# Photoroom/datago

Measured on AMD Instinct MI355X. Metric: Mpixel/s device-resident JPEG decode+bucket-resize at 1/2/4/8 MI355X, higher is better.
Workload: dtype u8

## Files before the change

datago_amd/csrc/dg_entropy.h:

```cpp
#pragma once
#include "dg_pixel.h"
#include "dg_plane.h"
#include "dg_types.h"

namespace dg {

DG_HD int32_t huff_extend(int32_t v, int32_t s) { return v < (1 << (s - 1)) ? v - (1 << s) + 1 : v; }

DG_HD uint32_t bswap32(uint32_t x) {
  return (x >> 24) | ((x >> 8) & 0xFF00u) | ((x << 8) & 0xFF0000u) | (x << 24);
}

DG_HD uint32_t ds_word_index(uint32_t w, uint32_t lsw) {
  const uint32_t s = w >> lsw, j = w & ((1u << lsw) - 1u);
  return ((((s >> 6) << lsw) + j) << 6) + (s & 63u);
}
DG_HD uint64_t ds_words_alloc(uint32_t nsub, uint32_t lsw) {
  const uint32_t margin = ((1024u >> 5) >> lsw) + 2u;
  return ((uint64_t)((nsub + margin + 63u) / 64u) << lsw) * 64;
}

constexpr uint32_t kBwBuf = 6;

struct BitWin {
// ... 369 lines not shown
}
DG_HD DG_GLOBAL uint32_t *stage_range(uint64_t stage, uint32_t cap, uint32_t s) {
  return (DG_GLOBAL uint32_t *)(uintptr_t)stage + ((((size_t)(s >> 6) * cap) << 6) + (s & 63u)) * 4;
}
DG_HD void stage_push(StageCtx &c, uint32_t e) {
  const uint32_t k = c.n & 3u;
  c.g0 = k == 0 ? e : c.g0;
  c.g1 = k == 1 ? e : c.g1;
  c.g2 = k == 2 ? e : c.g2;
  c.g3 = k == 3 ? e : c.g3;
  c.n++;
  if (k == 3) {
    DG_GLOBAL uint32_t *p = c.base + (size_t)((c.n >> 2) - 1) * 256;
#if defined(DG_DEVICE)
    *(DG_GLOBAL u32x4 *)p = u32x4{c.g0, c.g1, c.g2, c.g3};
#else
    p[0] = c.g0, p[1] = c.g1, p[2] = c.g2, p[3] = c.g3;
#endif
  }
}
DG_HD void stage_finish(StageCtx &c) {
  if (c.n & 3u) {
    DG_GLOBAL uint32_t *p = c.base + (size_t)(c.n >> 2) * 256;
#if defined(DG_DEVICE)
    *(DG_GLOBAL u32x4 *)p = u32x4{c.g0, c.g1, c.g2, c.g3};
#else
    p[0] = c.g0, p[1] = c.g1, p[2] = c.g2, p[3] = c.g3;
#endif
  }
}

constexpr uint32_t kCkptBits = 256;
constexpr uint32_t kMaxCkpt = 16;
template <int NC>
struct CkptN {
  uint32_t st;
  uint32_t m, n;
  int32_t dc[NC];
};
using Ckpt = CkptN<3>;

DG_HD uint32_t num_ckpt(uint32_t sub_bits) {
  uint32_t k = (sub_bits - 1) / kCkptBits;
  return k > kMaxCkpt ? kMaxCkpt : k;
}

DG_HD uint32_t first_marker(const DG_GLOBAL uint32_t *mk, uint32_t nmk, uint32_t pos, uint32_t &idx) {
  uint32_t lo = 0, hi = nmk;
  while (lo < hi) {
    uint32_t mid = (lo + hi) >> 1;
    if (mk[mid] < pos) lo = mid + 1;
    else hi = mid;
  }
  idx = lo;
  return lo < nmk ? mk[lo] : kInf;
}

template <class TAB>
DG_HD uint32_t lead_in(const ImageDesc &im, const TAB *tabs, const DG_GLOBAL uint8_t *stream,
                       const DG_GLOBAL uint32_t *mk, uint32_t s, uint32_t lead,
                       const uint16_t *mt = nullptr, uint32_t acm = 0xFFu, bool pair = false, uint32_t chain = 0) {
  const uint32_t a0 = s * im.sub_bits;
  if (s == 0 || lead == 0 || a0 >= im.ds_bits) return pack_state(0, 0, 0);
  uint32_t pos = a0 > lead ? a0 - lead : 0u;
  uint32_t r = 0, z = 0, midx;
  uint32_t mpos = im.nmk ? first_marker(mk, im.nmk, pos, midx) : kInf;
  const uint32_t bpm = im.bpm, slotmap = im.slotmap, cbits = im.comp_bits;
  uint32_t comp = cbits & 3u;
  const TAB *tdc = &tabs[(slotmap >> ((comp << 1) << 2)) & 15u];
  const TAB *tac = &tabs[(slotmap >> (((comp << 1) | 1u) << 2)) & 15u];
  uint32_t mi = mt ? (acm >> (2u * comp)) & 3u : 3u;
  BitWin b;
  bw_init(b, stream, im.ds_lsw, pos);
  for (;;) {
    if (pos >= mpos) {
      pos = mpos;
      r = 0;
// ... 127 lines not shown
          setn(acc.dc, 0);
          if (WRITE) {
            w->seg++;
            w->nin = 0;
            setn(w->pred, 0);
          }
        }
        midx++;
        mpos = midx < im.nmk ? mk[midx] : kInf;
        bw_seek(b, pos);
      }
      if (k < nck && cpos < a1 && pos >= cpos) {
        uint32_t rel = pos - cpos;
        uint32_t st = pack_state(rel > 255 ? 255 : rel, r, z);
        DG_GLOBAL CkptN<NC> &c = ck[k];
        if (merge && c.st == st) {
          if (c.m) {
            acc.m += c.m;
            acc.n = c.n;
            cpyn<NC>(acc.dc, c.dc);
          } else {
            acc.n += c.n;
            accn<NC>(acc.dc, c.dc);
          }
          acc.out = old_out;
          merged = true;
          break;
        }
        c.st = st;
        c.m = acc.m;
        c.n = acc.n;
        cpyn<NC>(c.dc, acc.dc);
        k++;
        cpos += kCkptBits;
      }
      if (pos >= a1) break;
      ev = next_event();
    }
    bw_refill(b);
    const uint32_t bits = bw_peek(b, pos);
    const bool isdc = (z == 0);
    const uint32_t e = huff_decode(*(isdc ? tdc : tac), bits);
    const uint32_t len = e >> 8, sym = e & 0xFFu;
    const uint32_t size = sym & 15u;
    const uint32_t run = isdc ? 0u : (sym >> 4);
    const int32_t v = huff_value(bits, len, size);
    uint32_t zm = 0xFFFFFFFFu, mc = 0;
    if (!WRITE) {
      const uint32_t m = (mi != 3u && !isdc) ? (uint32_t)mt[(mi << kMultiBits) | (bits >> (32u - kMultiBits))] : 0u;
      mc = m & 15u;
      zm = pos + mc <= ev ? multi_next_z(m, z) : 0xFFFFFFFFu;
    }
    const bool take_m = zm != 0xFFFFFFFFu;
    const uint32_t p0 = pos;
    pos += take_m ? mc : len + size;
    const int32_t vdc = isdc ? v : 0;
    acc.n += isdc ? 1u : 0u;
    addn(acc.dc, comp, vdc);
    if (stage) {
      if (isdc) {
        stg->started++;
        if (v) stage_push(*stg, stage_coef(0, stg->started, v));
      } else if (size && z + run < 64) {
        stage_push(*stg, stage_coef(z + run, stg->started, v));
      }
    }
    if (WRITE) {
// ... 309 lines not shown
```

datago_amd/csrc/dg_types.h:

```cpp
#pragma once
#include <stdint.h>

#if defined(__HIP__)
#define DG_HD __host__ __device__ __forceinline__
#define DG_DEVICE 1
#define DG_GLOBAL __attribute__((address_space(1)))
typedef unsigned int u32x4 __attribute__((ext_vector_type(4)));
typedef unsigned int u32x2 __attribute__((ext_vector_type(2)));
#else
#define DG_HD static inline
#define DG_GLOBAL
#endif

namespace dg {

template <class T>
DG_HD DG_GLOBAL T *gp(uint64_t a) {
  return (DG_GLOBAL T *)(uintptr_t)a;
}

DG_HD int32_t sel3(const int32_t v[3], uint32_t c) { return c == 0 ? v[0] : (c == 1 ? v[1] : v[2]); }
DG_HD void add3(int32_t v[3], uint32_t c, int32_t d) {
  v[0] += c == 0 ? d : 0;
  v[1] += c == 1 ? d : 0;
// ... 448 lines not shown
  uint32_t first;
  uint32_t next;
  uint64_t deps;
};
constexpr uint32_t kProgDone = 0xFFFFFFFFu;
constexpr uint32_t kProgNoScan = 0xFFFFFFFFu;
constexpr uint16_t kProgChained = 1;
constexpr uint32_t kProgMaxScans = 256;
constexpr uint32_t kProgMaxDepScans = 64;
constexpr uint32_t kProgZeroBytes = 65536;

struct WgItem {
  uint32_t image;
  uint32_t item0;
};

struct BatchFlags {
  uint32_t chain_changed;
  uint32_t fix_count;
  uint32_t write_mismatch;
  uint32_t sync_iters_max;
  uint32_t idct_late;
  uint32_t png_next;
  uint64_t wgtime;
  uint32_t wgtime_write;
  uint32_t debug;
  uint64_t idct_list;
  uint32_t idct_cap;
  uint32_t prio;
};
constexpr size_t kFlagCounters = 24;
constexpr uint32_t kDbgForceWriteMismatch = 1u;
constexpr uint32_t kDbgForceChainChange = 2u;

}
```

datago_amd/csrc/host/options.cpp:

```cpp
#include "options.h"

#include <string.h>

namespace dg {

static_assert(sizeof(size_t) == sizeof(uint64_t), "size_t fields are kOptU64");
static_assert(kMaxInflight == 6, "the texts of \"slots\" and \"coalesce_inflight\" spell it out");

namespace {

template <class T> constexpr OptType opt_type();
template <> constexpr OptType opt_type<bool>() { return kOptBool; }
template <> constexpr OptType opt_type<int>() { return kOptInt; }
template <> constexpr OptType opt_type<uint32_t>() { return kOptU32; }
template <> constexpr OptType opt_type<int64_t>() { return kOptI64; }
template <> constexpr OptType opt_type<uint64_t>() { return kOptU64; }
template <> constexpr OptType opt_type<double>() { return kOptDouble; }

constexpr int64_t kNoMax = INT64_MAX;

#define DG_STR2(x) #x
#define DG_STR(x) DG_STR2(x)
#define F(f) offsetof(Options, f), opt_type<decltype(Options::f)>()
#define FLAG(key, f) {key, F(f), kOptFlag, 0, 0, 0, 0, nullptr, kAfterNone}
// ... 66 lines not shown
    RANGE("decode_semantics", decode_sem, 0, 1, "valid unless v != 0 && v != 1"),
    RANGE("small_coded", small_coded, 0, kNoMax, "valid unless v < 0"),
    POW2("sub_small", sub_small, 64, 65536, "valid unless v < 64 || v > 65536 || (v & (v - 1))"),
    RANGE("lead_small", lead_small, 0, 1 << 16, "valid unless v < 0 || v > (1 << 16)"),
    POW2_OR_0("v_tile", v_tile, 2, 8, "valid: 0, 2, 4, 8"),
    RANGE("v_units", v_units, 1, 8, "valid unless v < 1 || v > 8"),
    RANGE("lead_big", lead_big, 0, 1 << 16, "valid unless v < 0 || v > (1 << 16)"),
    FLAG("write_split", write_split),
    RANGE("meta_pull", meta_pull, 0, 2, "valid unless v < 0 || v > 2"),
    RANGE("plan_threads", plan_threads, 1, 64, "valid unless v < 1 || v > 64"),
    POW2("inf_stage3", inf_stage3, 8, 64, "valid unless v != 8 && v != 16 && v != 32 && v != 64"),
    RANGE("inf_cap", inf_cap, 10, 100, "valid unless v < 10 || v > 100"),
    FLAG("png_alias", png_alias),
    RANGE("inf_pad", inf_pad, 0, 1 << 20, "valid unless v < 0 || v > 2^20"),
    POW2("inf_chunk", inf_chunk, 4096, 65536, "valid unless v < 4096 || v > 65536 || (v & (v - 1))"),
    {"png_chunked", F(chunked_off), kOptFlagInv, 0, 0, 0, 0, nullptr, kAfterNone},
    FLAG("lead_density", lead_density),
    RANGE("sub_density", sub_density, 0, 4096, "valid unless v < 0 || v > 4096"),
    RANGE("uf_per_cu", uf_per_cu, 0, 16, "valid unless v < 0 || v > 16"),
    RANGE("uf_units", uf_units, 1, 2, "valid unless v < 1 || v > 2"),
    {"inf_decode", F(inf_decode), kOptRangeBut, 0, 28, 10, 0, "valid unless v < 0 || v > 28 || v == 10", kAfterNone},
    FLAG("h_mfma", h_mfma),
    FLAG("band_dec", band_dec),
    RAW("dec_dbg", dec_dbg),
    RANGE("dec_strips", dec_strips, 1, 4096, "valid unless v < 1 || v > 4096"),
    RAW("debug_flags", debug_flags),
};
const int kNumOptions = (int)(sizeof(kOptionTable) / sizeof(kOptionTable[0]));

const OptRow kOptionTableAdded[] = {
    STRICT("webp_lossy", webp_lossy),
    STRICT("webp_alpha", webp_alpha),
    STRICT("bmp", bmp),
};
const int kNumOptionsAdded = (int)(sizeof(kOptionTableAdded) / sizeof(kOptionTableAdded[0]));

const OptRow *find_option(const char *key) {
  for (const OptRow &r : kOptionTable)
    if (!strcmp(r.name, key)) return &r;
  for (const OptRow &r : kOptionTableAdded)
    if (!strcmp(r.name, key)) return &r;
  return nullptr;
}

bool option_takes(const OptRow &r, int64_t v) {
  switch (r.kind) {
    case kOptRange: return v >= r.lo && v <= r.hi;
    case kOptRangeBut: return v >= r.lo && v <= r.hi && v != r.except;
    case kOptPow2: return v >= r.lo && v <= r.hi && !(v & (v - 1));
    case kOptPow2Or0: return v == 0 || (v >= r.lo && v <= r.hi && !(v & (v - 1)));
    default: return true;
  }
}

void store_option(const OptRow &r, Options &o, int64_t v) {
  void *p = (char *)&o + r.off;
  switch (r.type) {
    case kOptNone: break;
    case kOptBool: *(bool *)p = r.kind == kOptFlagInv ? v == 0 : v != 0; break;
    case kOptInt: *(int *)p = (int)v; break;
    case kOptU32: *(uint32_t *)p = (uint32_t)v; break;
    case kOptI64: *(int64_t *)p = v; break;
    case kOptU64: *(uint64_t *)p = (uint64_t)v << r.shift; break;
    case kOptDouble: *(double *)p = (double)v; break;
  }
}
// ... 21 lines not shown
```

datago_amd/csrc/host/options.h:

```cpp
#pragma once
#include <stddef.h>
#include <stdint.h>

#include <string>

#include "../dg_types.h"

namespace dg {

constexpr int kMaxInflight = 6;
#ifndef DG_PROG_SLOTS
#define DG_PROG_SLOTS 2
#endif
constexpr int kProgSlots = DG_PROG_SLOTS;

struct Options {
  uint32_t sub_bits = 0;
  uint32_t sub_auto = 8192;
  int64_t lead_bits = -1;
  uint32_t lead_big = 4096;
  uint64_t small_coded = 0;
  uint32_t sub_small = 512, lead_small = 1024;
  double sub_density = 0;
  bool lead_density = false;
  bool multi_lead = true;
  int write_pair = 3;
  bool sync2 = false;
  int sync_chain = 2;
  bool sync_pair = false;
  bool write_split = true;
  bool ckpt = true;
  int entropy_prio = 0;
  bool entropy_lpt = true;
  bool entropy_once = false;
  bool destuff_one = false;
  int decode_sem = 0;

  bool idct_fused = false;
  bool idct_thread = true;
  bool sparse_coef = true;
  bool chroma_rec = true;
  bool band_dec = false;
  uint32_t dec_dbg = 0;
  uint32_t dec_strips = kDecStripsDefault;
  uint32_t hb_bands = kHBandsDefault;
  bool hv_fused = false;
  bool h_prefetch = true;
  bool h_planar = true;
  bool h_mfma = false;
  uint32_t v_tile = 4;
  uint32_t v_units = 2;
  size_t ccache_cap = (size_t)256 << 20;

  bool chunked_off = false;
  uint32_t inf_chunk = kInfChunk;
  uint32_t inf_cap = 30;
  bool png_alias = true;
  uint32_t inf_pad = 65536;
  uint32_t inf_stage3 = 32;
  uint32_t inf_decode = 25;
  int uf_per_cu = 0;
  uint32_t uf_units = 1;

// ... 94 lines not shown
```

datago_amd/csrc/host/pipeline.cpp:

```cpp
#include "pipeline_util.h"

#include <string.h>

#include <algorithm>
#include <atomic>
#include <chrono>
#include <cmath>
#include <thread>

#include "../dg_entropy.h"
#include "../dg_pixel.h"
#include "../dg_vp8.h"
#include "../kernels.h"

namespace dg {

thread_local std::string g_last_error;
void set_error(const std::string &s) { g_last_error = s; }

static constexpr int kMaxResyncRounds = 64;

void parallel_copy(const std::vector<CopyJob> &jobs, int nthreads) {
  constexpr size_t kPiece = 1 << 20;
  std::vector<CopyJob> pieces;
// ... 293 lines not shown
    case kAfterResetHostUs:
      for (double &x : host_us_) x = 0;
      for (double &x : host_cpu_us_) x = 0;
      break;
    default:
      break;
  }
  return DG_OK;
}

int64_t Context::get_stat(const std::string &k) {
  if (k == "batches") return stat_batches_;
  if (k == "coalesced_batches") return stat_coalesced_batches_;
  if (k == "coalesced_images") return stat_coalesced_images_;
  if (k == "resync_rounds") return stat_resync_;
  if (k == "fix_workgroups") return stat_fix_;
  if (k == "write_mismatch") return stat_mismatch_;
  if (k == "unsettled_batches") return stat_unsettled_;
  if (k == "prog_items") return stat_prog_items_;
  if (k == "prog_aggregates") return stat_prog_aggs_;
  if (k == "prog_aggregate_images") return stat_prog_agg_images_;
  if (k == "prog_chains") return stat_prog_chains_;
  if (k == "pool_flushes") return stat_pool_flush_;
  if (k == "sync_iters_max") return stat_iters_;
  if (k == "sync_chain") return opt_.sync_chain;
  {
    static const char *kn[2] = {"sync", "write"}, *sn[4] = {"span", "mean", "p90", "max"};
    for (int a = 0; a < 2; a++)
      for (int q = 0; q < 4; q++)
        if (k == std::string("wg_") + kn[a] + "_" + sn[q]) return (int64_t)(wgstat_[a][q] * 1000.0);
  }
  if (k == "sub_bits") return last_sub_bits_;
  if (k == "sub_auto") return opt_.sub_auto;
  if (k == "coalesce_inflight") return opt_.coalesce_inflight;
  if (k == "meta_bytes") return (int64_t)last_meta_bytes_;
  if (k == "allocs") return stat_allocs_;
  if (k == "alloc_mb") return stat_alloc_mb_;
  if (k == "alloc_us") return (int64_t)stat_alloc_us_;
  if (k == "reclaims") return stat_reclaims_;
  if (k == "peak_device_mb") return stat_peak_dev_ >> 20;
  if (k == "device_mb") {
    std::lock_guard<std::mutex> lk(mu_);
    return (int64_t)(dev_footprint() >> 20);
  }
  if (k == "max_device_mb") return (int64_t)(opt_.max_dev_bytes >> 20);
  if (k == "budget_splits") return stat_budget_splits_;
  if (k == "budget_plan_mb") return (int64_t)(plan_arena_ >> 20);
  if (k == "budget_slots") return opt_.max_dev_bytes ? std::min<int64_t>(opt_.nslots, stat_budget_slots_min_) : opt_.nslots;
  if (k == "coef_cache_hits") return stat_ccache_hits_;
  if (k == "coef_cache_new") return stat_ccache_new_;
  if (k == "coef_cache_resets") return stat_ccache_resets_;
  if (k == "coef_cache_mb") return (int64_t)(ccache_off_ >> 20);
  if (k == "budget_frees") return stat_budget_frees_;
  if (k == "budget_oom") return stat_budget_oom_;
  if (k == "retire_syncs") return stat_retire_syncs_;
  if (k == "png_serial_fallbacks") return stat_png_serial_;
  if (k == "band_dec_images") return stat_band_dec_;
  if (k == "direct_d2h") return stat_direct_d2h_;
  if (k == "png_chunks") return stat_png_chunks_;
  if (k == "png_small_streams") return stat_png_small_;
  {
    static const char *pn[8] = {"plan", "pools", "layout", "lists", "upload", "h2d", "launch", "slotwait"};
    for (int q = 0; q < 8; q++) {
      if (k == std::string("host_us_") + pn[q]) return (int64_t)host_us_[q];
      if (q < 7 && k == std::string("host_cpu_us_") + pn[q]) return (int64_t)host_cpu_us_[q];
    }
// ... 922 lines not shown
  if (!from_fix && !b.pscans.empty()) {
    hipStream_t pst = pside ? sl.side : sl.st;
    launch_prog_zero(pst, dd, lst(L_PROG_ZERO), cnt(L_PROG_ZERO));
    const ProgScan *ps = (const ProgScan *)(M + b.pscan_off);
    const uint32_t prog_dbg = ((uint32_t)(opt_.debug_flags >> 19) & 1u) << 1;
    uint64_t *pt = b.ptime_off ? (uint64_t *)((char *)sl.wgt.p + b.ptime_off) : nullptr;
    if (opt_.prog_pipe) {
      uint32_t *pf = (uint32_t *)((char *)sl.scratch.p + b.pf_off);
      HIPCHK(hipMemsetAsync(pf, 0, (size_t)(b.pf_n + 2) * 4, pst));
      const uint32_t nac = cnt(L_PROG) - b.prog_dc_n, sflags = (opt_.prog_serial ? 1u : 0u) | prog_dbg;
      hipStream_t dst = pst;
      if (!pside && opt_.side_stream && b.prog_dc_n && nac) {
        HIPCHK(hipEventRecord(sl.ev_zero, pst));
        HIPCHK(hipStreamWaitEvent(sl.side, sl.ev_zero, 0));
        dst = sl.side;
        dc_side = true;
      }
      launch_prog_scan(pst, dd, ps, lst(L_PROG), nac, hp, sflags, pf, pf, pt, 1);
      launch_prog_scan(dst, dd, ps, lst(L_PROG) + nac, b.prog_dc_n, hp, sflags, pf, pf + b.pf_n + 1, pt, 4);
      if (dc_side) HIPCHK(hipEventRecord(sl.ev_prog, sl.side));
    } else {
      uint32_t at = 0;
      for (uint32_t nl : b.prog_level_n) {
        launch_prog_scan(pst, dd, ps, lst(L_PROG) + at, nl, hp, opt_.prog_serial ? 1u : 0u, nullptr, nullptr, pt, 4);
        at += nl;
      }
    }
    if (pside) HIPCHK(hipEventRecord(sl.ev_prog, sl.side));
  }
  if (next()) return DG_ERR_DEVICE;
  Ckpt *ck = (Ckpt *)((char *)sl.scratch.p + sl.ckpt_off);
  if (!from_fix)
    launch_huff_sync(sl.st, dd, lst(L_SYNC), cnt(L_SYNC), hp, subs, ck, fl, b.stage_on, b.max_slots,
                     opt_.multi_lead ? b.max_ac : 0u, opt_.sync_pair, opt_.sync2, (uint32_t)opt_.sync_chain, b.nc4);
  if (next()) return DG_ERR_DEVICE;
  launch_huff_fix(sl.st, dd, lst(L_SYNC), cnt(L_SYNC), hp, subs, ck, fl, b.stage_on, b.max_slots, b.nc4);
  if (next()) return DG_ERR_DEVICE;
  launch_huff_scan(sl.st, dm, lst(L_SCAN), cnt(L_SCAN), subs, b.nc4);
  if (next()) return DG_ERR_DEVICE;
  launch_ms_zero(sl.st, dd, lst(L_MS_ZERO), cnt(L_MS_ZERO));
  if (b.stage_on)
    launch_huff_scatter(sl.st, dd, lst(L_HUFF), cnt(L_HUFF), subs);
  else
    launch_huff_write(sl.st, dm, lst(L_HUFF), cnt(L_HUFF), hp, subs, fl, b.max_slots, qp, (uint32_t)opt_.write_pair, ck,
                      b.nc4, b.ms);
  if (next()) return DG_ERR_DEVICE;
  if (next()) return DG_ERR_DEVICE;
  if (pside || dc_side) HIPCHK(hipStreamWaitEvent(sl.st, sl.ev_prog, 0));
  if (b.any_fused) launch_idct_list(sl.st, dd, qp, fl, std::min<uint32_t>(2048u, (b.idct_cap + 31) / 32));
  if (opt_.idct_thread)
    launch_idct_t(sl.st, dd, lst(L_IDCT), cnt(L_IDCT), qp);
  else
    launch_idct(sl.st, dd, lst(L_IDCT), cnt(L_IDCT), qp);
  if (next()) return DG_ERR_DEVICE;
  launch_color(sl.st, dd, lst(L_COLOR), cnt(L_COLOR));
  launch_cmyk(sl.st, dd, lst(L_CMYK), cnt(L_CMYK));
  if (next()) return DG_ERR_DEVICE;
  HIPCHK(hipStreamWaitEvent(sl.st, sl.ev_coef, 0));
  launch_alpha(sl.st, dd, lst(L_ALPHA0), cnt(L_ALPHA0), 0 | (alpha_flags << 8));
  launch_band_dec(sl.st, dd, lst(L_DEC), b.decclass, qp, opt_.dec_strips | (opt_.dec_dbg << 16));
  launch_resize_hm(sl.st, dd, lst(L_RM0), b.hmclass[0], 0);
  launch_resize_hb(sl.st, dd, lst(L_RH0), b.hclass[0], 0, opt_.h_prefetch, opt_.h_planar, b.h_zune != 0);
  launch_resize_hv(sl.st, dd, lst(L_RHV), b.hvclass);
  launch_resize_h(sl.st, dd, lst(L_RHX0), cnt(L_RHX0), 0 | ((opt_.debug_flags & 0xFF) << 8));
  if (!from_fix) launch_r16_v(sl.st, dd, lst(L_R16V), cnt(L_R16V));
  if (next()) return DG_ERR_DEVICE;
  launch_resize_v(sl.st, dd, lst(L_RV1), cnt(L_RV1), 1, opt_.v_units);
// ... 677 lines not shown
```

datago_amd/csrc/host/pipeline.h:

```cpp
#pragma once
#include <hip/hip_runtime.h>

#include <chrono>
#include <memory>
#include <condition_variable>
#include <mutex>
#include <string>
#include <unordered_map>
#include <vector>

#include "../../../include/datago_hip.h"
#include "../dg_types.h"
#include "../dg_resize16.h"
#include "buckets.h"
#include "options.h"
#include "jpeg_header.h"
#include "gif_header.h"
#include "bmp_header.h"
#include "webp_header.h"
#include "png_header.h"
#include "jpeg_enc.h"
#include "host_pool.h"

namespace dg {
// ... 47 lines not shown
  std::vector<ImagePlan> plans;
  std::vector<ImageDesc> descs;
  std::vector<int> desc_of;
  std::vector<WgItem> lists[55];
  size_t list_off[55] = {0};
  std::vector<GatherJob> gjobs;
  size_t gjob_off = 0;
  std::vector<InfChunk> ichunks;
  size_t ichunk_off = 0;
  uint32_t uf_n = 0;
  uint32_t uf_maxbpp = 1;
  size_t uf_flags_off = 0;
  uint32_t ds_n = 0;
  size_t ds_state_off = 0;
  uint32_t pf_n = 0;
  size_t pf_off = 0;
  size_t ptime_off = 0;
  uint32_t prog_dc_n = 0;
  std::vector<uint8_t> blob;
  size_t blob_off = 0;
  bool any_png = false, any_alpha = false, any_enc = false;
  bool any_gif = false;
  bool any_webp = false;
  bool any_alph = false;
  bool any_bmp = false;
  bool any_vp8 = false;
  bool penc_dyn = false;
  bool jenc_opt = false;
  bool any_fused = false;
  uint32_t idct_cap = 0;
  uint32_t v_tile = 0;
  uint32_t h_zune = 0;
  bool stage_on = false;
  bool nc4 = false;
  bool ms = false;
  struct MsScan {
    int desc, parent;
    int image, scan;
  };
  std::vector<MsScan> ms_scans;
  struct AlphStream {
    int desc, parent;
    int image;
  };
  std::vector<AlphStream> alph_streams;
  uint32_t max_slots = 1;
  uint32_t max_ac = 0;
  size_t words_off = 0, words_bytes = 0;
  size_t enctab_off = 0;
  std::vector<ProgScan> pscans;
  size_t pscan_off = 0;
  std::vector<uint32_t> prog_level_n;
  uint32_t hclass[2][2][4] = {{{0}}};
  uint32_t hvclass[2] = {0, 0};
  uint32_t decclass[2] = {0, 0};
  uint32_t hmclass[2][2][2] = {{{0}}};
  size_t desc_off = 0, flags_off = 0;
  size_t meta_bytes = 0;
  size_t total_subs = 0;
  std::vector<uint8_t *> host_outs;
  std::vector<uint64_t> host_caps;
  std::vector<size_t> out_dev_off;
  std::vector<uint8_t> out_direct;
  std::vector<dg_payload_meta *> mptr;
  std::vector<dg_payload_meta> local_meta;
  std::vector<dg_payload_meta *> pub;
// ... 315 lines not shown
```

datago_amd/csrc/host/submit.cpp:

```cpp
#include <string.h>
#include <time.h>

#include <algorithm>
#include <chrono>
#include <cmath>

#include "../dg_alph.h"
#include "../dg_entropy.h"
#include "../dg_bmp.h"
#include "../dg_gif.h"
#include "../dg_vp8.h"
#include "../dg_vp8l.h"
#include "../dg_jenc_tree.h"
#include "../dg_pixel.h"
#include "../kernels.h"
#include "pipeline_util.h"

namespace dg {

static double thread_cpu_us() {
  timespec ts;
  clock_gettime(CLOCK_THREAD_CPUTIME_ID, &ts);
  return (double)ts.tv_sec * 1e6 + (double)ts.tv_nsec * 1e-3;
}
// ... 680 lines not shown
  }
  d.nslots = (uint8_t)nslots;
  b.max_slots = std::max<uint32_t>(b.max_slots, (uint32_t)nslots);
  if (!h.progressive && !h.multiscan) {
    uint32_t acs = 0;
    for (int c = 0; c < h.ncomp; c++) acs |= 1u << ((d.slotmap >> ((2 * c + 1) * 4)) & 15u);
    b.max_ac = std::max<uint32_t>(b.max_ac, std::min<uint32_t>((uint32_t)__builtin_popcount(acs), kMultiLuts));
  }
  if (h.progressive) {
    d.prog = (uint32_t)h.scans.size();
    if (a.host_io) bl.in_off[i] = bl.IN.take(a.lens[i] + 16, 16);
  } else if (h.multiscan) {
    d.ms.role = kMsParent;
    if (a.host_io) bl.in_off[i] = bl.IN.take(a.lens[i] + 16, 16);
  } else {
    layout_entropy(a, i, b, bl, d, o);
  }
  o.coef = bl.CO.take((size_t)d.total_blocks * 128);
  o.ccnt = (opt_.sparse_coef && opt_.idct_thread && !d.prog && !d.idct_fused && !(opt_.entropy_once && !b.nc4 && !b.ms))
               ? bl.CO.take((size_t)d.total_blocks, 64) + 1
               : 0;
  for (int c = 0; c < 4; c++) o.plane[c] = (size_t)-1;
  if (h.ncomp >= 3) d.pix_stride = (uint32_t)align_up((size_t)W * 3, 16);
}

void Context::layout_entropy(const SubmitArgs &a, int i, Batch &b, BatchLayout &bl, ImageDesc &d, Offs &o) {
  const JpegHeader &h = b.plans[i].hdr;
  layout_entropy_stream(h.scan_end - h.scan_off, b, bl, d, o);
  if (a.host_io) bl.in_off[i] = bl.IN.take(a.lens[i] + 16, 16);
}

void Context::layout_entropy_stream(size_t scan_len, Batch &b, BatchLayout &bl, ImageDesc &d, Offs &o) {
  const uint32_t sub_bits = bl.sub_bits;
  const bool once = opt_.entropy_once && !b.nc4 && !b.ms;
  d.scan_len = (uint32_t)scan_len;
  d.sub_bits = sub_bits;
  if (opt_.sub_density > 0 && opt_.sub_bits == 0) {
    const double bpb = (double)d.scan_len * 8.0 / (double)std::max<uint32_t>(1, d.total_blocks);
    if (bpb < opt_.sub_density * 0.5 && sub_bits >= 2048)
      d.sub_bits = sub_bits / 4;
    else if (bpb < opt_.sub_density && sub_bits >= 1024)
      d.sub_bits = sub_bits / 2;
  }
  d.idct_fused = (opt_.idct_fused && !once && !b.nc4 && !b.ms) ? 1u : 0u;
  if (opt_.write_split && d.ckpt && !d.idct_fused && !once && d.restart == 0 && d.sub_bits >= 1024 &&
      d.sub_bits / 2 / kCkptBits - 1 < num_ckpt(d.sub_bits))
    d.ckpt |= 2u;
  if (d.idct_fused) b.any_fused = true;
  d.lead_bits = opt_.lead_bits >= 0 ? (uint32_t)opt_.lead_bits : bl.small ? opt_.lead_small : (d.bpm >= 4 ? opt_.lead_big : 2048u);
  if (opt_.lead_density && opt_.lead_bits < 0 && d.sub_bits < sub_bits)
    d.lead_bits = std::max<uint32_t>(1024u, d.lead_bits / (sub_bits / d.sub_bits));
  d.nsub = std::max<uint32_t>(1, (uint32_t)(((uint64_t)d.scan_len * 8 + d.sub_bits - 1) / d.sub_bits));
  d.sub_base = bl.sub_base;
  bl.sub_base += d.nsub;
  d.ckpt_base = (uint32_t)bl.ckpt_total;
  bl.ckpt_total += (uint64_t)d.nsub * num_ckpt(d.sub_bits);
  d.nchunk = std::max<uint32_t>(1, (d.scan_len + kDestuffChunk - 1) / kDestuffChunk);
  const uint32_t mcus = d.total_blocks / d.bpm;
  d.mk_cap = (d.restart ? mcus / d.restart + 2 : 0) + 64;
  d.ds_lsw = 0;
  while ((32u << d.ds_lsw) < d.sub_bits) d.ds_lsw++;
  o.ds = bl.L.take((size_t)ds_words_alloc(d.nsub, d.ds_lsw) * 4, 256);
  if (once && d.sub_bits <= 8192) {
    d.stage_cap = (d.sub_bits / 2 + d.sub_bits / 8 + 64 + 3) / 4;
    o.stage = bl.L.take((size_t)((d.nsub + 63) / 64) * d.stage_cap * 64 * 16, 256);
    b.stage_on = true;
  }
  o.mk = bl.L.take((size_t)d.mk_cap * 4, 16);
  o.chunk = bl.L.take((size_t)d.nchunk * 16, 16);
}

int Context::plan_resize(const ImagePlan &p, Batch &b, BatchLayout &bl, ImageDesc &d, Offs &o) {
  const uint32_t W = d.width, H = d.height, C = d.dec_c;
  const bool colour = p.fmt == kFmtJpeg && d.ncomp == 3;
  size_t cur_stride = decoded_stride(d);
  d.out_w = p.out_w;
  d.out_h = p.out_h;
  d.out_c = p.out_c;
  d.out_stride = p.out_w * p.out_c * (p.bit_depth == 16 ? 2 : 1);
  if (p.r16) return plan_resize16(p, bl, d, o);
  uint32_t cw = W, chh = H;
// ... 642 lines not shown
    for (size_t lv = 1; lv < at.size(); lv++) at[lv] = at[lv - 1] + b.prog_level_n[lv - 1];
    b.lists[L_PROG].resize(b.pscans.size());
    for (uint32_t j = 0; j < (uint32_t)b.pscans.size(); j++)
      b.lists[L_PROG][at[b.pscans[j].level]++] = WgItem{b.pscans[j].image, j};
  }
  for (int c = 0; c < 2; c++) {
    b.decclass[c] = (uint32_t)cl.decl[c].size();
    b.lists[L_DEC].insert(b.lists[L_DEC].end(), cl.decl[c].begin(), cl.decl[c].end());
  }
  for (int c = 0; c < 2; c++) {
    b.hvclass[c] = (uint32_t)cl.hvl[c].size();
    b.lists[L_RHV].insert(b.lists[L_RHV].end(), cl.hvl[c].begin(), cl.hvl[c].end());
  }
  for (int h = 0; h < 2; h++)
    for (int f = 1; f >= 0; f--)
      for (int k = 0; k < 2; k++) {
        b.hmclass[h][f][k] = (uint32_t)cl.hm[h][f][k].size();
        auto &l = b.lists[h ? L_RM2 : L_RM0];
        l.insert(l.end(), cl.hm[h][f][k].begin(), cl.hm[h][f][k].end());
      }
  for (int h = 0; h < 2; h++)
    for (int f = 1; f >= 0; f--)
      for (int c = 0; c < 4; c++) {
        b.hclass[h][f][c] = (uint32_t)cl.hb[h][f][c].size();
        auto &l = b.lists[h ? L_RH2 : L_RH0];
        l.insert(l.end(), cl.hb[h][f][c].begin(), cl.hb[h][f][c].end());
      }
}

void Context::image_items(int di, Batch &b, ClassLists &cl) {
  const ImageDesc &d = b.descs[di];
  const uint32_t I = (uint32_t)di;
  auto entropy_items = [&]() {
    const uint32_t wstep = (d.ckpt & 2u) ? kSubPerWg / 2 : kSubPerWg;
    for (uint32_t w = 0; w < d.nsub; w += wstep) b.lists[L_HUFF].push_back({I, w});
    for (uint32_t w = 0; w < d.nsub; w += kSubPerWg - 1) b.lists[L_SYNC].push_back({I, w});
    b.descs[di].ds_state0 = (uint32_t)b.lists[L_DESTUFF].size();
    for (uint32_t c = 0; c < d.nchunk; c++) b.lists[L_DESTUFF].push_back({I, c});
    for (uint32_t c = 0; c < d.nchunk; c += kDsWgChunks) b.lists[L_DESTUFF_WG].push_back({I, c});
    b.lists[L_SCAN].push_back({I, 0});
  };
  if (d.ms.role == kMsScan) {
    entropy_items();
    return;
  }
  for (uint32_t k = 0; k < kAlphaPoints; k++)
    if (d.aop[k].prog) {
      const uint32_t cnt = d.aop[k].width * d.aop[k].rows;
      for (uint32_t it = 0; it < cnt; it += 256) b.lists[L_ALPHA0 + k].push_back({I, it});
    }
  if (d.fmt == kFmtWebp && !d.dec_c) {
    b.lists[L_VP8L].push_back({I, 0});
    return;
  }
  if (d.fmt == kFmtVp8) {
    b.lists[L_VP8].push_back({I, 0});
    if (d.dec_c == 4)
      for (uint32_t it = 0; it < alph_items(d.vp8.alph_filter, d.width, d.height); it++) b.lists[L_ALPH].push_back({I, it});
    for (uint32_t it = 0; it < d.width * d.height; it += 256) b.lists[L_VP8_RGB].push_back({I, it});
  } else if (d.fmt == kFmtWebp) {
    b.lists[L_VP8L].push_back({I, 0});
    for (uint32_t it = 0; it < d.width * d.height; it += 256) b.lists[L_VP8L_STORE].push_back({I, it});
  } else if (d.fmt == kFmtBmp) {
    if (d.bmp.rle) b.lists[L_BMP_RLE].push_back({I, 0});
    for (uint32_t it = 0; it < bmp_row_groups(d.width) * d.height; it += 64) b.lists[L_BMP_EXPAND].push_back({I, it});
  } else if (d.fmt == kFmtGif) {
    b.lists[L_GIF_LZW].push_back({I, 0});
// ... 105 lines not shown
  b.desc_off = M.take(b.descs.size() * sizeof(ImageDesc));
  for (int l = 0; l < L_COUNT; l++) b.list_off[l] = M.take(b.lists[l].size() * sizeof(WgItem));
  b.gjob_off = M.take(b.gjobs.size() * sizeof(GatherJob));
  b.ichunk_off = M.take(b.ichunks.size() * sizeof(InfChunk));
  b.pscan_off = M.take(b.pscans.size() * sizeof(ProgScan));
  b.blob_off = M.take(b.blob.size());
  b.meta_bytes = align_up(M.off, 256);
  dg_status st = ensure(sl.meta, b.meta_bytes + 256, sl.st);
  if (st) return st;
  for (ImageDesc &d : b.descs) {
    if (d.fmt == kFmtPng && d.png.pal) d.png.pal = (uint64_t)(uintptr_t)((char *)sl.meta.p + b.blob_off + d.png.pal - 1);
    if (d.fmt == kFmtBmp && d.bmp.pal) d.bmp.pal = (uint64_t)(uintptr_t)((char *)sl.meta.p + b.blob_off + d.bmp.pal - 1);
    if (d.fmt == kFmtGif) d.gif.pal = (uint64_t)(uintptr_t)((char *)sl.meta.p + b.blob_off + d.gif.pal - 1);
    if (d.enc.active) {
      d.enc.hdr = (uint64_t)(uintptr_t)((char *)sl.meta.p + b.blob_off + d.enc.hdr - 1);
      if (!d.enc.png) d.enc.tab = d.enc.tab_std = (uint64_t)(uintptr_t)((char *)sl.meta.p + b.blob_off + b.enctab_off);
    }
  }
  size_t stage_bytes = b.meta_bytes + (a.host_io ? bl.IN.off : 0);
  st = ensure_pinned(sl.stage, stage_bytes + 256, sl.st);
  if (st) return st;
  char *P = (char *)sl.stage.p;
  memset(P + b.flags_off, 0, sizeof(BatchFlags));
  b.ptime_off = 0;
  if (opt_.wg_timing) {
    const size_t nrec = b.lists[L_SYNC].size() + b.lists[L_HUFF].size();
    b.ptime_off = b.pscans.empty() ? 0 : nrec * 16 + 64;
    st = ensure(sl.wgt, nrec * 16 + 64 + b.pscans.size() * 16, sl.st);
    if (st) return st;
    BatchFlags *bf = (BatchFlags *)(P + b.flags_off);
    bf->wgtime = (uint64_t)(uintptr_t)sl.wgt.p;
    bf->wgtime_write = (uint32_t)b.lists[L_SYNC].size();
  }
  ((BatchFlags *)(P + b.flags_off))->debug = (uint32_t)(opt_.debug_flags >> 16) & 3u;
  ((BatchFlags *)(P + b.flags_off))->prio = (uint32_t)opt_.entropy_prio;
  ((BatchFlags *)(P + b.flags_off))->idct_list = (uint64_t)(uintptr_t)((char *)sl.scratch.p + bl.idct_list_off);
  ((BatchFlags *)(P + b.flags_off))->idct_cap = b.idct_cap;
  memcpy(P + b.desc_off, b.descs.data(), b.descs.size() * sizeof(ImageDesc));
  for (int l = 0; l < L_COUNT; l++)
    if (!b.lists[l].empty()) memcpy(P + b.list_off[l], b.lists[l].data(), b.lists[l].size() * sizeof(WgItem));
  if (!b.gjobs.empty()) memcpy(P + b.gjob_off, b.gjobs.data(), b.gjobs.size() * sizeof(GatherJob));
  if (!b.ichunks.empty()) memcpy(P + b.ichunk_off, b.ichunks.data(), b.ichunks.size() * sizeof(InfChunk));
  if (!b.pscans.empty()) memcpy(P + b.pscan_off, b.pscans.data(), b.pscans.size() * sizeof(ProgScan));
  if (!b.blob.empty()) memcpy(P + b.blob_off, b.blob.data(), b.blob.size());
  if (a.host_io) {
    std::vector<CopyJob> ins;
    for (int i = 0; i < a.n; i++)
      if (b.desc_of[i] >= 0) ins.push_back({P + b.meta_bytes + bl.in_off[i], a.h_srcs[i], a.lens[i]});
    parallel_copy(ins, opt_.copy_threads);
  }
  last_meta_bytes_ = b.meta_bytes;
  return DG_OK;
}

dg_status Context::enqueue_upload(const SubmitArgs &a, Slot &sl, Batch &b, const BatchLayout &bl) {
  char *P = (char *)sl.stage.p;
  if (opt_.timing) HIPCHK(hipEventRecord(sl.ev[0], sl.st));
  if (opt_.meta_pull >= 1) {
    launch_meta_pull(sl.st, P, sl.meta.p, b.meta_bytes);
    HIPCHK(hipGetLastError());
  } else {
    HIPCHK(hipMemcpyAsync(sl.meta.p, P, b.meta_bytes, hipMemcpyHostToDevice, sl.st));
  }
  if (a.host_io && bl.IN.off) {
    if (opt_.meta_pull >= 2) {
      launch_meta_pull(sl.st, P + b.meta_bytes, sl.input.p, bl.IN.off);
      HIPCHK(hipGetLastError());
// ... 20 lines not shown
```

datago_amd/csrc/kernels.hip:

```cpp
#include <hip/hip_runtime.h>

#include "dg_destuff.h"
#include "dg_entropy.h"
#include "dg_pixel.h"
#include "dg_plane.h"
#include "kernels.h"

#pragma clang fp contract(off)

namespace dg {


__device__ __forceinline__ void load_tables(HuffTable *tabs, const HuffTable *pool, const ImageDesc &im) {
  const int words = (int)(sizeof(HuffTable) / 4);
  const int ns = im.nslots;
  for (int i = threadIdx.x; i < ns * words; i += blockDim.x) {
    int s = i / words, w = i - s * words;
    ((uint32_t *)&tabs[s])[w] = ((const uint32_t *)&pool[im.hslot[s]])[w];
  }
}

__device__ __forceinline__ uint32_t xcd_remap(uint32_t b, uint32_t n) {
  const uint32_t per = n >> 3, rem = n & 7, x = b & 7, l = b >> 3;
  return x * per + (x < rem ? x : rem) + l;
// ... 778 lines not shown
}

constexpr int kBlkStride = 64;

template <int NC, bool MS = false>
__global__ __launch_bounds__(256) void k_huff_write(ImageDesc *__restrict__ imgs,
                                                    const WgItem *__restrict__ list,
                                                    const HuffTable *__restrict__ pool,
                                                    const SubState *__restrict__ subs, BatchFlags *flags,
                                                    const QuantTable *__restrict__ qpool, uint32_t pair,
                                                    const Ckpt *__restrict__ ckpt) {
  extern __shared__ __attribute__((aligned(16))) uint8_t huff_dyn[];
  HuffTable *tabs = (HuffTable *)huff_dyn;
  __shared__ __attribute__((aligned(16))) int16_t blk[kSubPerWg][kBlkStride];
  __shared__ uint32_t wtab[kSubPerWg / 64][128];
  __shared__ int32_t qt[3 * 64];
  __shared__ uint8_t n2z[64];
  const uint64_t t_start = wg_clock();
  entropy_setprio(flags);
  const WgItem it = list[blockIdx.x];
  const ImageDesc &im = imgs[it.image];
  load_tables(tabs, pool, im);
  const bool fused = im.idct_fused != 0;
  if (fused) {
    const int t = threadIdx.x;
    if (t < 64) n2z[kZigzagToNatural[t]] = (uint8_t)t;
    if (t < 3 * 64 && (uint32_t)(t >> 6) < im.ncomp) {
      const DG_GLOBAL uint16_t *q = gp<const uint16_t>((uint64_t)(uintptr_t)qpool[im.qpool[t >> 6]].q);
      qt[t] = q[t & 63];
    }
  }
  __syncthreads();
  const int t = threadIdx.x;
  const bool split = (im.ckpt & 2u) != 0;
  const uint32_t s = split ? it.item0 + (uint32_t)(t & 63) + ((uint32_t)(t >> 7) << 6) : it.item0 + (uint32_t)t;
  const uint32_t half = split ? ((uint32_t)t >> 6) & 1u : 0u;
  bool run = s < im.nsub;
  uint32_t in = 0, want = 0, a0o = kInf, a1o = kInf;
  SubState ss = {};
  if (run) {
    ss = subs[im.sub_base + s];
    in = ss.in;
    want = ss.out;
    if (split) {
      const uint32_t S = im.sub_bits, mid = s * S + S / 2, kmid = S / 2 / kCkptBits - 1;
      const CkptN<NC> c = ((const CkptN<NC> *)ckpt)[im.ckpt_base + (size_t)s * num_ckpt(S) + kmid];
      const bool ok = mid < im.ds_bits && im.nmk == 0 && ss.m == 0 && c.m == 0 && st_rel(c.st) < 255u;
      if (!ok) {
        run = half == 0;
      } else if (half == 0) {
        a1o = mid;
        want = c.st;
      } else {
        a0o = mid;
        in = c.st;
        ss.nin += ss.n - c.n;
        ss.dcin[0] += ss.dc[0] - c.dc[0];
        ss.dcin[1] += ss.dc[1] - c.dc[1];
        ss.dcin[2] += ss.dc[2] - c.dc[2];
        if (NC == 4) ss.dcin[NC - 1] += ss.dc[NC - 1] - c.dc[NC - 1];
      }
    }
  }
  if (run) {
    WriteCtxN<NC> w;
    w.blk = blk[t];
    w.sw = (((uint32_t)t >> 1) & 7u) << 3;
    w.coef = gp<int16_t>(im.coef);
    w.seg = ss.seg;
    w.nin = ss.nin;
    cpyn<NC>(w.pred, ss.dcin);
    w.blocks_per_seg = im.blocks_per_seg;
    w.total_blocks = im.total_blocks;
    w.cur = -1;
    w.zs = 0;
    w.cnt = (im.ccnt && !fused) ? gp<uint8_t>(im.ccnt) : nullptr;
    w.wave_blk = blk[t & ~63];
    w.stride = kBlkStride;
    w.tab = wtab[t >> 6];
    w.im = fused ? &im : nullptr;
    w.qt = qt;
    w.n2z = n2z;
    w.flags = flags;
    w.img = it.image;
    {
      u32x4 *p = (u32x4 *)w.blk;
      const u32x4 zero = {0u, 0u, 0u, 0u};
#pragma unroll
      for (int i = 0; i < 8; i++) p[i] = zero;
    }
    RangeAccN<NC> acc;
    decode_range<true, HuffTable, true, NC, MS>(im, tabs, gp<const uint8_t>(im.ds), gp<const uint32_t>(im.mk), s, in,
                                                acc, &w, nullptr, false, 0, nullptr, nullptr, 0xFFu, pair, a0o, a1o);
    if (acc.out != want || (s == 0 && (flags->debug & kDbgForceWriteMismatch))) {
      atomicAdd(&flags->write_mismatch, 1u);
// ... 2432 lines not shown
```

Baseline: 141,500.

## Generalize write-phase split from halves to up to 16 checkpointed pieces per subsequence

Replaces the fixed two-way split of each entropy subsequence's write pass with a K-way split (default scaled by sub_bits/4096, capped at 16). Each piece starts from a stored checkpoint, so more threads decode one subsequence in parallel. For long subsequences, checkpoints beyond the dense 256-bit region are stored every 2048 bits. It also disables entropy_once and sync2 for long subs. The cost is more workgroups, more checkpoint reads, and fallback to whole-piece decoding when a checkpoint is unusable.

```diff
diff --git a/datago_amd/csrc/dg_entropy.h b/datago_amd/csrc/dg_entropy.h
--- a/datago_amd/csrc/dg_entropy.h
+++ b/datago_amd/csrc/dg_entropy.h
@@ -425,6 +425,8 @@
 
 constexpr uint32_t kCkptBits = 256;
 constexpr uint32_t kMaxCkpt = 16;
+constexpr uint32_t kCkptFarBits = 2048;
+constexpr uint32_t kCkptDenseSub = 8192;
 template <int NC>
 struct CkptN {
   uint32_t st;
@@ -435,7 +437,59 @@
 
 DG_HD uint32_t num_ckpt(uint32_t sub_bits) {
   uint32_t k = (sub_bits - 1) / kCkptBits;
+  if (sub_bits > kCkptDenseSub) return kMaxCkpt + (sub_bits - kMaxCkpt * kCkptBits - 1) / kCkptFarBits;
   return k > kMaxCkpt ? kMaxCkpt : k;
+}
+DG_HD uint32_t ckpt_step(uint32_t sub_bits, uint32_t k) {
+  return (sub_bits > kCkptDenseSub && k >= kMaxCkpt) ? kCkptFarBits : kCkptBits;
+}
+DG_HD int32_t ckpt_at(uint32_t sub_bits, uint32_t off) {
+  const uint32_t nck = num_ckpt(sub_bits), dense = kMaxCkpt * kCkptBits;
+  uint32_t k;
+  if (off == 0 || off >= sub_bits) return -1;
+  if (off <= dense || sub_bits <= kCkptDenseSub) {
+    if (off % kCkptBits) return -1;
+    k = off / kCkptBits - 1;
+  } else {
+    if ((off - dense) % kCkptFarBits) return -1;
+    k = kMaxCkpt - 1 + (off - dense) / kCkptFarBits;
+  }
+  return k < nck ? (int32_t)k : -1;
+}
+
+template <int NC>
+DG_HD bool write_piece_plan(const ImageDesc &im, const CkptN<NC> *ckr, uint32_t s, uint32_t lgk,
+                            uint32_t piece, bool merge_dbg, SubState &ss, uint32_t &in, uint32_t &want,
+                            uint32_t &a0o, uint32_t &a1o) {
+  in = ss.in;
+  want = ss.out;
+  a0o = kInf;
+  a1o = kInf;
+  if (lgk == 0) return true;
+  const uint32_t S = im.sub_bits, r0 = s * S, step = S >> lgk, K = 1u << lgk;
+  const bool whole = im.nmk != 0 || ss.m != 0;
+  CkptN<NC> c;
+  auto piece_start = [&](uint32_t q) -> bool {
+    const int32_t k = ckpt_at(S, q * step);
+    if (whole || k < 0 || r0 + q * step >= im.ds_bits) return false;
+    if (merge_dbg && (q & 1u) && !(s & 1u)) return false;
+    c = ckr[k];
+    return c.m == 0 && st_rel(c.st) < 255u;
+  };
+  if (piece > 0) {
+    if (!piece_start(piece)) return false;
+    a0o = r0 + piece * step;
+    in = c.st;
+    ss.nin += ss.n - c.n;
+    for (int i = 0; i < NC; i++) ss.dcin[i] += ss.dc[i] - c.dc[i];
+  }
+  for (uint32_t q = piece + 1; q < K; q++)
+    if (piece_start(q)) {
+      a1o = r0 + q * step;
+      want = c.st;
+      break;
+    }
+  return true;
 }
 
 DG_HD uint32_t first_marker(const DG_GLOBAL uint32_t *mk, uint32_t nmk, uint32_t pos, uint32_t &idx) {
@@ -629,7 +683,7 @@
         c.n = acc.n;
         cpyn<NC>(c.dc, acc.dc);
         k++;
-        cpos += kCkptBits;
+        cpos += ckpt_step(S, k);
       }
       if (pos >= a1) break;
       ev = next_event();
diff --git a/datago_amd/csrc/dg_types.h b/datago_amd/csrc/dg_types.h
--- a/datago_amd/csrc/dg_types.h
+++ b/datago_amd/csrc/dg_types.h
@@ -504,5 +504,6 @@
 constexpr size_t kFlagCounters = 24;
 constexpr uint32_t kDbgForceWriteMismatch = 1u;
 constexpr uint32_t kDbgForceChainChange = 2u;
-
-}
+constexpr uint32_t kDbgForceWriteMerge = 4u;
+
+}
diff --git a/datago_amd/csrc/host/options.cpp b/datago_amd/csrc/host/options.cpp
--- a/datago_amd/csrc/host/options.cpp
+++ b/datago_amd/csrc/host/options.cpp
@@ -122,6 +122,7 @@
     STRICT("webp_lossy", webp_lossy),
     STRICT("webp_alpha", webp_alpha),
     STRICT("bmp", bmp),
+    {"write_pieces", F(write_pieces), kOptPow2Or0, 1, 16, 0, 0, "valid: 0, 1, 2, 4, 8, 16", kAfterNone},
 };
 const int kNumOptionsAdded = (int)(sizeof(kOptionTableAdded) / sizeof(kOptionTableAdded[0]));
 
diff --git a/datago_amd/csrc/host/options.h b/datago_amd/csrc/host/options.h
--- a/datago_amd/csrc/host/options.h
+++ b/datago_amd/csrc/host/options.h
@@ -29,6 +29,7 @@
   int sync_chain = 2;
   bool sync_pair = false;
   bool write_split = true;
+  uint32_t write_pieces = 0;
   bool ckpt = true;
   int entropy_prio = 0;
   bool entropy_lpt = true;
diff --git a/datago_amd/csrc/host/pipeline.cpp b/datago_amd/csrc/host/pipeline.cpp
--- a/datago_amd/csrc/host/pipeline.cpp
+++ b/datago_amd/csrc/host/pipeline.cpp
@@ -349,6 +349,7 @@
   }
   if (k == "sub_bits") return last_sub_bits_;
   if (k == "sub_auto") return opt_.sub_auto;
+  if (k == "write_pieces") return opt_.write_pieces;
   if (k == "coalesce_inflight") return opt_.coalesce_inflight;
   if (k == "meta_bytes") return (int64_t)last_meta_bytes_;
   if (k == "allocs") return stat_allocs_;
@@ -1337,7 +1338,7 @@
   Ckpt *ck = (Ckpt *)((char *)sl.scratch.p + sl.ckpt_off);
   if (!from_fix)
     launch_huff_sync(sl.st, dd, lst(L_SYNC), cnt(L_SYNC), hp, subs, ck, fl, b.stage_on, b.max_slots,
-                     opt_.multi_lead ? b.max_ac : 0u, opt_.sync_pair, opt_.sync2, (uint32_t)opt_.sync_chain, b.nc4);
+                     opt_.multi_lead ? b.max_ac : 0u, opt_.sync_pair, opt_.sync2 && !b.long_sub, (uint32_t)opt_.sync_chain, b.nc4);
   if (next()) return DG_ERR_DEVICE;
   launch_huff_fix(sl.st, dd, lst(L_SYNC), cnt(L_SYNC), hp, subs, ck, fl, b.stage_on, b.max_slots, b.nc4);
   if (next()) return DG_ERR_DEVICE;
diff --git a/datago_amd/csrc/host/pipeline.h b/datago_amd/csrc/host/pipeline.h
--- a/datago_amd/csrc/host/pipeline.h
+++ b/datago_amd/csrc/host/pipeline.h
@@ -103,6 +103,7 @@
   uint32_t v_tile = 0;
   uint32_t h_zune = 0;
   bool stage_on = false;
+  bool long_sub = false;
   bool nc4 = false;
   bool ms = false;
   struct MsScan {
diff --git a/datago_amd/csrc/host/submit.cpp b/datago_amd/csrc/host/submit.cpp
--- a/datago_amd/csrc/host/submit.cpp
+++ b/datago_amd/csrc/host/submit.cpp
@@ -736,7 +736,7 @@
 
 void Context::layout_entropy_stream(size_t scan_len, Batch &b, BatchLayout &bl, ImageDesc &d, Offs &o) {
   const uint32_t sub_bits = bl.sub_bits;
-  const bool once = opt_.entropy_once && !b.nc4 && !b.ms;
+  const bool once = opt_.entropy_once && !b.nc4 && !b.ms && sub_bits <= 8192;
   d.scan_len = (uint32_t)scan_len;
   d.sub_bits = sub_bits;
   if (opt_.sub_density > 0 && opt_.sub_bits == 0) {
@@ -747,10 +747,17 @@
       d.sub_bits = sub_bits / 2;
   }
   d.idct_fused = (opt_.idct_fused && !once && !b.nc4 && !b.ms) ? 1u : 0u;
-  if (opt_.write_split && d.ckpt && !d.idct_fused && !once && d.restart == 0 && d.sub_bits >= 1024 &&
-      d.sub_bits / 2 / kCkptBits - 1 < num_ckpt(d.sub_bits))
-    d.ckpt |= 2u;
+  uint32_t pieces = opt_.write_pieces ? opt_.write_pieces
+                    : !opt_.write_split ? 1u
+                                        : std::min(16u, std::max(2u, d.sub_bits / 4096u));
+  while (pieces > 1 && d.sub_bits / pieces < 512) pieces /= 2;
+  if (pieces > 1 && d.ckpt && !d.idct_fused && !once && d.restart == 0 && ckpt_at(d.sub_bits, d.sub_bits / 2) >= 0) {
+    uint32_t lg = 0;
+    while ((1u << lg) < pieces) lg++;
+    d.ckpt |= lg << 1;
+  }
   if (d.idct_fused) b.any_fused = true;
+  if (sub_bits > 8192) b.long_sub = true;
   d.lead_bits = opt_.lead_bits >= 0 ? (uint32_t)opt_.lead_bits : bl.small ? opt_.lead_small : (d.bpm >= 4 ? opt_.lead_big : 2048u);
   if (opt_.lead_density && opt_.lead_bits < 0 && d.sub_bits < sub_bits)
     d.lead_bits = std::max<uint32_t>(1024u, d.lead_bits / (sub_bits / d.sub_bits));
@@ -1459,7 +1466,7 @@
   const ImageDesc &d = b.descs[di];
   const uint32_t I = (uint32_t)di;
   auto entropy_items = [&]() {
-    const uint32_t wstep = (d.ckpt & 2u) ? kSubPerWg / 2 : kSubPerWg;
+    const uint32_t wstep = (uint32_t)kSubPerWg >> ((d.ckpt >> 1) & 7u);
     for (uint32_t w = 0; w < d.nsub; w += wstep) b.lists[L_HUFF].push_back({I, w});
     for (uint32_t w = 0; w < d.nsub; w += kSubPerWg - 1) b.lists[L_SYNC].push_back({I, w});
     b.descs[di].ds_state0 = (uint32_t)b.lists[L_DESTUFF].size();
@@ -1631,7 +1638,8 @@
     bf->wgtime = (uint64_t)(uintptr_t)sl.wgt.p;
     bf->wgtime_write = (uint32_t)b.lists[L_SYNC].size();
   }
-  ((BatchFlags *)(P + b.flags_off))->debug = (uint32_t)(opt_.debug_flags >> 16) & 3u;
+  ((BatchFlags *)(P + b.flags_off))->debug =
+      ((uint32_t)(opt_.debug_flags >> 16) & 3u) | (((uint32_t)(opt_.debug_flags >> 20) & 1u) << 2);
   ((BatchFlags *)(P + b.flags_off))->prio = (uint32_t)opt_.entropy_prio;
   ((BatchFlags *)(P + b.flags_off))->idct_list = (uint64_t)(uintptr_t)((char *)sl.scratch.p + bl.idct_list_off);
   ((BatchFlags *)(P + b.flags_off))->idct_cap = b.idct_cap;
diff --git a/datago_amd/csrc/kernels.hip b/datago_amd/csrc/kernels.hip
--- a/datago_amd/csrc/kernels.hip
+++ b/datago_amd/csrc/kernels.hip
@@ -834,35 +834,25 @@
   }
   __syncthreads();
   const int t = threadIdx.x;
-  const bool split = (im.ckpt & 2u) != 0;
-  const uint32_t s = split ? it.item0 + (uint32_t)(t & 63) + ((uint32_t)(t >> 7) << 6) : it.item0 + (uint32_t)t;
-  const uint32_t half = split ? ((uint32_t)t >> 6) & 1u : 0u;
+  const uint32_t lgk = (im.ckpt >> 1) & 7u, K = 1u << lgk;
+  const uint32_t per_wg = (uint32_t)kSubPerWg >> lgk;
+  uint32_t piece, sl;
+  if (per_wg >= 64u) {
+    const uint32_t wv = (uint32_t)t >> 6;
+    piece = wv & (K - 1u);
+    sl = ((wv >> lgk) << 6) + ((uint32_t)t & 63u);
+  } else {
+    piece = (uint32_t)t / per_wg;
+    sl = (uint32_t)t & (per_wg - 1u);
+  }
+  const uint32_t s = it.item0 + sl;
   bool run = s < im.nsub;
   uint32_t in = 0, want = 0, a0o = kInf, a1o = kInf;
   SubState ss = {};
   if (run) {
     ss = subs[im.sub_base + s];
-    in = ss.in;
-    want = ss.out;
-    if (split) {
-      const uint32_t S = im.sub_bits, mid = s * S + S / 2, kmid = S / 2 / kCkptBits - 1;
-      const CkptN<NC> c = ((const CkptN<NC> *)ckpt)[im.ckpt_base + (size_t)s * num_ckpt(S) + kmid];
-      const bool ok = mid < im.ds_bits && im.nmk == 0 && ss.m == 0 && c.m == 0 && st_rel(c.st) < 255u;
-      if (!ok) {
-        run = half == 0;
-      } else if (half == 0) {
-        a1o = mid;
-        want = c.st;
-      } else {
-        a0o = mid;
-        in = c.st;
-        ss.nin += ss.n - c.n;
-        ss.dcin[0] += ss.dc[0] - c.dc[0];
-        ss.dcin[1] += ss.dc[1] - c.dc[1];
-        ss.dcin[2] += ss.dc[2] - c.dc[2];
-        if (NC == 4) ss.dcin[NC - 1] += ss.dc[NC - 1] - c.dc[NC - 1];
-      }
-    }
+    run = write_piece_plan<NC>(im, (const CkptN<NC> *)ckpt + im.ckpt_base + (size_t)s * num_ckpt(im.sub_bits), s, lgk,
+                               piece, (flags->debug & kDbgForceWriteMerge) != 0, ss, in, want, a0o, a1o);
   }
   if (run) {
     WriteCtxN<NC> w;
```

Result: no change. 140,900 (-0.5%).
